# facebookresearch/multipathnet

Hardware: AMD Instinct MI355X
Metric: proposals/sec (1000 ROIs, 600x1000 img) VGG-16 Fast R-CNN (higher is better)
Workload: dtype f32; 1 GPU; VGG-16 Fast R-CNN, 1 image 600x1000 x 1000 ROIs per GPU per step, 21 classes, NMS 0.3, top-100 (BASELINE configs[1]); host image + boxes uploaded inside the step (pinned, copy stream, three staging sets)

## Files before the change

multipathnet_amd/csrc/dense.hip:

```cpp
#include <cstdlib>
#include <type_traits>
#include <vector>

#include "dense.h"

namespace mpn {

typedef float f32x16 __attribute__((ext_vector_type(16)));
typedef float f32x4 __attribute__((ext_vector_type(4)));

#define MPN_GPTR(p) ((const __attribute__((address_space(1))) void *)(p))
#define MPN_LPTR(p) ((__attribute__((address_space(3))) void *)(p))

__device__ __forceinline__ void glds16(const float *gsrc, float *lds_wave_base) {
  __builtin_amdgcn_global_load_lds(MPN_GPTR(gsrc), MPN_LPTR(lds_wave_base), 16, 0, 0);
}

__device__ __forceinline__ void glds16_saddr(const float *base_uniform, unsigned lane_byte_off, unsigned lds_byte_addr_uniform) {
  asm volatile("s_mov_b32 m0, %0\n\ts_nop 0\n\tglobal_load_lds_dwordx4 %1, %2"
               :
               : "s"(lds_byte_addr_uniform), "v"(lane_byte_off), "s"(base_uniform)
               : "memory");
}
__device__ __forceinline__ void dma_wait_all() { asm volatile("s_waitcnt vmcnt(0)" ::: "memory"); }
// ... 101 lines not shown
    if (MPN_ABLATE(a.ablate & 4)) {
#pragma unroll
      for (int mi = 0; mi < MI; ++mi) af[1][mi] = af[0][mi];
#pragma unroll
      for (int ni = 0; ni < NI; ++ni) bf[1][ni] = bf[0][ni];
    }
#pragma unroll
    for (int t = 0; t < TPS; ++t) {
      const int cur = t & 1;
      if (t + 1 < TPS && !MPN_ABLATE(a.ablate & 4)) {
        const int nt = t + 1, dy = (TPS == 9) ? nt / 3 : 0, dx = nt % 3;
#pragma unroll
        for (int mi = 0; mi < MI; ++mi) af[cur ^ 1][mi] = *reinterpret_cast<const f32x4 *>(Wl + (nt * BM + mbase + mi * 32) * 8);
#pragma unroll
        for (int ni = 0; ni < NI; ++ni) bf[cur ^ 1][ni] = *reinterpret_cast<const f32x4 *>(Il + ((rbase + ni + dy) * 34 + dx) * 8);
      }
      if (more) {
#pragma unroll
        for (int k = 0; k < PER_TAP; ++k) issue_item(q + 1, t * PER_TAP + k);
      }
      __builtin_amdgcn_sched_barrier(0);
#pragma unroll
      for (int j = 0; j < 4; ++j)
#pragma unroll
        for (int mi = 0; mi < MI; ++mi)
#pragma unroll
          for (int ni = 0; ni < NI; ++ni)
            acc[mi][ni] = __builtin_amdgcn_mfma_f32_32x32x2f32(af[cur][mi][j], bf[cur][ni][j], acc[mi][ni], 0, 0, 0);
      __builtin_amdgcn_sched_barrier(0);
    }
    if (!MPN_ABLATE(a.ablate & 2)) __syncthreads();
  }

  const int x = x0 + l31;
  const bool xok = x < a.W;
  if (a.splits > 1) {
    float *pb = a.part + (size_t)blockIdx.y * a.part_slab;
#pragma unroll
    for (int mi = 0; mi < MI; ++mi)
#pragma unroll
      for (int g = 0; g < 4; ++g) {
        const int cb = (cout0 + mbase + mi * 32) / 8 + g;
        if (cb >= a.out_cb) continue;
#pragma unroll
        for (int ni = 0; ni < NI; ++ni) {
          const int y = y0 + rbase + ni;
          if (xok && y < a.H) {
            f32x4 v;
#pragma unroll
            for (int e = 0; e < 4; ++e) v[e] = acc[mi][ni][g * 4 + e];
            *reinterpret_cast<f32x4 *>(pb + (size_t)cb * a.out_plane + ((size_t)(y + 1) * a.out_Wp + x + 1) * 8 + half * 4) = v;
          }
        }
      }
    return;
  }
  if (MPN_ABLATE(a.ablate & 8)) {
    if (a.H < 0) {
#pragma unroll
      for (int mi = 0; mi < MI; ++mi)
#pragma unroll
        for (int ni = 0; ni < NI; ++ni) *reinterpret_cast<f32x16 *>(a.part + (size_t)(mi * NI + ni) * 16 + lane * 64) = acc[mi][ni];
    }
    return;
  }
#pragma unroll
  for (int mi = 0; mi < MI; ++mi) {
#pragma unroll
    for (int g = 0; g < 4; ++g) {
      const int cb = (cout0 + mbase + mi * 32) / 8 + g;
      if (cb >= a.out_cb) continue;
      const f32x4 b4 = *reinterpret_cast<const f32x4 *>(a.bpk + cb * 8 + half * 4);
      f32x4 v[NI];
#pragma unroll
      for (int ni = 0; ni < NI; ++ni) {
        const int y = y0 + rbase + ni;
        const bool ok = xok && (y < a.H);
#pragma unroll
        for (int e = 0; e < 4; ++e) {
          float t = acc[mi][ni][g * 4 + e] + b4[e];
          if (a.relu) t = t < 0.0f ? 0.0f : t;
          v[ni][e] = t;
        }
        if (ok && a.out)
          *reinterpret_cast<f32x4 *>(a.out + (size_t)cb * a.out_plane + ((size_t)(y + 1) * a.out_Wp + x + 1) * 8 + half * 4) = v[ni];
        if (!ok) v[ni] = f32x4{-INFINITY, -INFINITY, -INFINITY, -INFINITY};
      }
      if constexpr (NI % 2 == 0) {
        if (a.pool) {
#pragma unroll
          for (int q = 0; q < NI / 2; ++q) {
            f32x4 m;
#pragma unroll
            for (int e = 0; e < 4; ++e) {
              float t = fmaxf(v[2 * q][e], v[2 * q + 1][e]);
              t = fmaxf(t, __shfl_xor(t, 1));
              m[e] = t > -INFINITY ? t : -INFINITY;
            }
            const int py = ((y0 + rbase) >> 1) + q, px = x >> 1;
            if (!(l31 & 1) && py < a.pool_H && px < a.pool_W)
              *reinterpret_cast<f32x4 *>(a.pool + (size_t)cb * a.pool_plane + ((size_t)(py + 1) * a.pool_Wp + px + 1) * 8 + half * 4) = m;
          }
        }
      }
    }
  }
}

MPN_KNOB(int, g_gemm_ablate, 0);

constexpr int kF_TH = 8;
constexpr int kF_PL = (kF_TH + 2) * 34 + 12;
template <int ABL>
__global__ __launch_bounds__(256, 5) void conv3x3_first_kernel(const float *__restrict__ in, int in_Wp, const float *__restrict__ w36,
                                                               int CoutP, const float *__restrict__ bpk, float *__restrict__ out,
                                                               size_t out_plane, int out_Wp, int H, int W, int out_cb, int relu,
                                                               int tiles_x, int n_tiles) {
  __shared__ float tile[2][4 * kF_PL];
  __shared__ float wl[36 * 64];
  __shared__ float bl[64];
  const int tid = threadIdx.x, lane = tid & 63;
  const int wave = __builtin_amdgcn_readfirstlane(tid >> 6);
  const int half = lane >> 5, l31 = lane & 31;
  const int cout0 = blockIdx.y * 64;
  for (int i = tid; i < 36 * 64; i += 256) wl[i] = w36[(size_t)(i >> 6) * CoutP + cout0 + (i & 63)];
  if (tid < 64) bl[tid] = bpk[cout0 + tid];
  constexpr int NPX = (kF_TH + 2) * 34;
  const int p0 = tid, p1 = tid + 256;
  const int r0 = p0 / 34, c0 = p0 - r0 * 34, r1 = p1 / 34, c1 = p1 - r1 * 34;
  const int off0 = (r0 * in_Wp + c0) * 8, off1 = p1 < NPX ? (r1 * in_Wp + c1) * 8 : off0;
  auto fetch = [&](int t, f32x4 &v0, f32x4 &v1) {
    const int ty = t / tiles_x, tx = t - ty * tiles_x;
    const float *base = in + ((size_t)(ty * kF_TH) * in_Wp + tx * 32) * 8;
    v0 = *reinterpret_cast<const f32x4 *>(base + off0);
    v1 = *reinterpret_cast<const f32x4 *>(base + off1);
  };
  auto park = [&](int buf, const f32x4 &v0, const f32x4 &v1) {
#pragma unroll
    for (int e = 0; e < 4; ++e) tile[buf][e * kF_PL + p0] = v0[e];
    if (p1 < NPX) {
#pragma unroll
      for (int e = 0; e < 4; ++e) tile[buf][e * kF_PL + p1] = v1[e];
    }
  };
  int t = blockIdx.x;
  if (t >= n_tiles) return;
  const int step = gridDim.x;
  f32x4 n0, n1;
  fetch(t, n0, n1);
  park(0, n0, n1);
  if (t + step < n_tiles) fetch(t + step, n0, n1);
  __syncthreads();
  const float *wa = wl + half * 64 + l31;
  int buf = 0;
  for (; t < n_tiles; t += step, buf ^= 1) {
    const int ty = t / tiles_x, tx = t - ty * tiles_x;
    const int y0 = ty * kF_TH, x0 = tx * 32;
    const float *tb = tile[buf] + half * kF_PL + (wave * 2) * 34 + l31;
    const int x = x0 + l31;
    bool xok = x < W;
    if constexpr ((ABL & 1) != 0) xok = xok && in_Wp == 7;
    const int yw = y0 + wave * 2;
    const unsigned voff = (unsigned)(((yw + 1) * out_Wp + x + 1) * 8 + half * 4) * 4u;
    const unsigned vrow = (unsigned)out_Wp * 32u;
    const bool ok0 = xok && yw < H, ok1 = xok && yw + 1 < H;
#pragma unroll
    for (int mi = 0; mi < 2; ++mi) {
      f32x16 acc[2];
#pragma unroll
      for (int ni = 0; ni < 2; ++ni)
#pragma unroll
        for (int r = 0; r < 16; ++r) acc[ni][r] = 0.0f;
#pragma unroll
      for (int tp = 0; tp < 9; ++tp) {
        const int dy = tp / 3, dx = tp - dy * 3;
#pragma unroll
        for (int p = 0; p < 2; ++p) {
          const float afr = wa[(tp * 2 + p) * 128 + mi * 32];
          float bfr[2];
#pragma unroll
          for (int ni = 0; ni < 2; ++ni) bfr[ni] = tb[2 * p * kF_PL + (ni + dy) * 34 + dx];
#pragma unroll
          for (int ni = 0; ni < 2; ++ni) {
            if constexpr ((ABL & 2) == 0) acc[ni] = __builtin_amdgcn_mfma_f32_32x32x2f32(afr, bfr[ni], acc[ni], 0, 0, 0);
            else acc[ni][(tp + p) & 15] += afr * bfr[ni];
          }
        }
        if ((tp % 3) == 2) __builtin_amdgcn_sched_barrier(0);
      }
      if (mi == 1) {
        const int tn = t + step;
        if (tn < n_tiles) {
          park(buf ^ 1, n0, n1);
          if (tn + step < n_tiles) fetch(tn + step, n0, n1);
        }
        __builtin_amdgcn_sched_barrier(0);
      }
#pragma unroll
      for (int g = 0; g < 4; ++g) {
        const int cb = __builtin_amdgcn_readfirstlane((cout0 + mi * 32) / 8 + g);
        if (cb >= out_cb) continue;
        const f32x4 b4 = *reinterpret_cast<const f32x4 *>(bl + (mi * 4 + g) * 8 + half * 4);
        char *pb = reinterpret_cast<char *>(out + (size_t)cb * out_plane);
#pragma unroll
        for (int ni = 0; ni < 2; ++ni) {
          f32x4 v;
#pragma unroll
          for (int e = 0; e < 4; ++e) {
            float tv = acc[ni][g * 4 + e] + b4[e];
            if (relu) tv = tv < 0.0f ? 0.0f : tv;
            v[e] = tv;
          }
          if (ni ? ok1 : ok0) *reinterpret_cast<f32x4 *>(pb + (voff + (ni ? vrow : 0u))) = v;
        }
      }
      __builtin_amdgcn_sched_barrier(0);
    }
    __syncthreads();
  }
}

__global__ void pack_conv_w_first_kernel(const float *__restrict__ w, int Cin, int Cout, int CoutP, float *__restrict__ w36) {
  const int t = blockIdx.x * blockDim.x + threadIdx.x;
  if (t >= 36 * CoutP) return;
  const int row = t / CoutP, co = t - row * CoutP;
  const int hf = row & 1, ks = row >> 1, p = ks & 1, tap = ks >> 1;
  const int cin = 2 * p + hf;
  w36[t] = (co < Cout && cin < Cin) ? w[((size_t)co * Cin + cin) * 9 + tap] : 0.0f;
}

size_t conv_first_elems(int Cout) { return (size_t)36 * conv_coutp(Cout); }

int pack_conv_weights_first(const float *d_w, int Cin, int Cout, float *d_w36, hipStream_t s) {
  MPN_CHECK_ARG(d_w && d_w36 && Cin > 0 && Cin <= 4 && Cout > 0);
  const int CoutP = conv_coutp(Cout);
  hipLaunchKernelGGL(pack_conv_w_first_kernel, dim3(cdiv(36 * CoutP, 256)), dim3(256), 0, s, d_w, Cin, Cout, CoutP, d_w36);
  MPN_CHECK_LAUNCH();
  return MPN_OK;
}

int conv3x3_first_c8p(Act in, const float *d_w36, const float *d_bpk, int Cout, int relu, Act out, hipStream_t s) {
  MPN_CHECK_ARG(in.p && d_w36 && d_bpk && out.p && in.C <= 4 && out.H == in.H && out.W == in.W && out.C == Cout);
  const int tiles_x = cdiv(in.W, 32), tiles_y = cdiv(in.H, kF_TH), n_ct = cdiv(Cout, 64);
  const int n_tiles = tiles_x * tiles_y;
  const char *e_cap = MPN_ABLATE(1) ? getenv("MPN_FIRST_BLOCKS") : nullptr;
  const int cap = e_cap ? atoi(e_cap) : 1280;
  const int blocks = cdiv(n_tiles, cdiv(n_tiles, cap));
  auto kern = conv3x3_first_kernel<0>;
#ifdef MPN_DEBUG_HOOKS
  if ((g_gemm_ablate & 3) == 1) kern = conv3x3_first_kernel<1>;
  if ((g_gemm_ablate & 3) == 2) kern = conv3x3_first_kernel<2>;
  if ((g_gemm_ablate & 3) == 3) kern = conv3x3_first_kernel<3>;
#endif
  hipLaunchKernelGGL(kern, dim3((unsigned)blocks, (unsigned)n_ct), dim3(256), 0, s, in.p, in.Wp, d_w36, conv_coutp(Cout), d_bpk, out.p,
                     out.plane(), out.Wp, in.H, in.W, (Cout + 7) / 8, relu, tiles_x, n_tiles);
  MPN_CHECK_LAUNCH();
  return MPN_OK;
}

template <int BM, int TH, int WM, int WN, int TPS>
static int launch_conv(const ConvArgs &a0, int tiles_y, hipStream_t s) {
  ConvArgs a = a0;
  constexpr int IN_LOADS = ((TH + 2) * 68 + 63) / 64;
  constexpr size_t LDS = (size_t)2 * (IN_LOADS * 256 + TPS * BM * 8) * sizeof(float);
  auto kern = conv3x3_c8p_kernel<BM, TH, WM, WN, TPS>;
  { int rc_attr = set_max_dyn_lds(reinterpret_cast<const void *>(kern), (int)LDS); if (rc_attr) return rc_attr; }
  dim3 grid((unsigned)(a.n_ct * tiles_y * a.tiles_x), (unsigned)a.splits);
  hipLaunchKernelGGL(kern, grid, dim3(256), LDS, s, a);
  MPN_CHECK_LAUNCH();
  return MPN_OK;
}


typedef float f32x2 __attribute__((ext_vector_type(2)));
__device__ __forceinline__ f32x2 pk_sub(f32x2 a, f32x2 b) {
  f32x2 r;
  asm("v_pk_add_f32 %0, %1, %2 neg_lo:[0,1] neg_hi:[0,1]" : "=v"(r) : "v"(a), "v"(b));
  return r;
}
__device__ __forceinline__ f32x2 vmax_2(f32x2 a, f32x2 b) {
  f32x2 r;
  asm("v_max_f32 %0, %1, %2" : "=v"(r[0]) : "v"(a[0]), "v"(b[0]));
  asm("v_max_f32 %0, %1, %2" : "=v"(r[1]) : "v"(a[1]), "v"(b[1]));
  return r;
}
__device__ __forceinline__ f32x2 vrelu_2(f32x2 a) {
  f32x2 r;
  asm("v_max_f32 %0, 0, %1" : "=v"(r[0]) : "v"(a[0]));
  asm("v_max_f32 %0, 0, %1" : "=v"(r[1]) : "v"(a[1]));
  return r;
}
__device__ __forceinline__ f32x2 vmax3_2(f32x2 a, f32x2 b, f32x2 c) {
  f32x2 r;
  asm("v_max3_f32 %0, %1, %2, %3" : "=v"(r[0]) : "v"(a[0]), "v"(b[0]), "v"(c[0]));
  asm("v_max3_f32 %0, %1, %2, %3" : "=v"(r[1]) : "v"(a[1]), "v"(b[1]), "v"(c[1]));
  return r;
}
__device__ __forceinline__ f32x2 vmax3_2s(f32x2 a, f32x2 b, float c_uniform) {
  f32x2 r;
  asm("v_max3_f32 %0, %1, %2, %3" : "=v"(r[0]) : "v"(a[0]), "v"(b[0]), "s"(c_uniform));
  asm("v_max3_f32 %0, %1, %2, %3" : "=v"(r[1]) : "v"(a[1]), "v"(b[1]), "s"(c_uniform));
  return r;
}
constexpr int WG_RAW_LOADS = 12;
constexpr int WG_RAW_FLOATS = WG_RAW_LOADS * 256;
constexpr int WG_V_FLOATS = 16 * 64 * 8;
constexpr int WG_U_FLOATS = 16 * 64 * 8;
constexpr size_t WG_LDS_BYTES = (size_t)2 * (WG_RAW_FLOATS + WG_V_FLOATS + WG_U_FLOATS) * sizeof(float);

template <int ABL, int TC>
__global__ __launch_bounds__(256) void conv3x3_wino_kernel(ConvArgs a) {
  constexpr int TR = 64 / TC;
  constexpr int RC = 2 * TC + 2, RR = 2 * TR + 2;
  constexpr int WG_RAW_PIECES = RR * RC * 2;
  static_assert((WG_RAW_PIECES + 63) / 64 <= WG_RAW_LOADS, "raw tile DMA slots");
  extern __shared__ __attribute__((aligned(16))) float lds[];
  float *const raw_lds = lds;
  float *const v_lds = lds + 2 * WG_RAW_FLOATS;
  float *const u_lds = v_lds + 2 * WG_V_FLOATS;
  const int tid = threadIdx.x, lane = tid & 63;
  unsigned long long tk0 = 0, tk1 = 0, tk2 = 0;
  if constexpr ((ABL & 64) != 0) tk0 = __builtin_amdgcn_s_memtime();
  const int wave = __builtin_amdgcn_readfirstlane(tid >> 6);
  const int half = lane >> 5, l31 = lane & 31;
  int bid = blockIdx.x, split = blockIdx.y, cps = a.chunks_per_split;
  bool partial = a.splits > 1;
  if (a.tail_splits > 1 && bid >= a.tail_first) {
    const int t = bid - a.tail_first;
    split = t % a.tail_splits; bid = a.tail_first + t / a.tail_splits; cps = a.tail_cps; partial = true;
  }
  const int ct = bid % a.n_ct, sp = bid / a.n_ct;
  const int tyb = sp / a.tiles_x, txb = sp - tyb * a.tiles_x;
  const int y0 = tyb * (2 * TR), x0 = txb * (2 * TC), cout0 = ct * 64;
  const int mbase = (wave >> 1) * 32, nbase = (wave & 1) * 32;

  constexpr int RAW_IT = (WG_RAW_LOADS + 3) / 4;
  unsigned raw_rel[RAW_IT];
#pragma unroll
  for (int i = 0; i < RAW_IT; ++i) {
    int p = min((i * 4 + wave) * 64 + lane, WG_RAW_PIECES - 1);
    int r = p / (RC * 2), o = p - r * (RC * 2);
    raw_rel[i] = (unsigned)(((r * a.in_Wp) * 8 + o * 4) * 4);
  }
  const unsigned u_lane = (unsigned)((((wave & 1) * 64 + lane) * 4) * 4);
  const size_t u_chunk = (size_t)16 * a.CoutP * 8;
  const float *const in_tile = a.in + (size_t)(y0 * a.in_Wp + x0) * 8;
  const float *const w_tile = a.wpk + (size_t)cout0 * 8;
  const unsigned lds0 = lds_byte_addr(lds);
  const unsigned raw_slot = lds0 + (unsigned)(wave * 256) * 4, u_slot = lds0 + (unsigned)(2 * WG_RAW_FLOATS + 2 * WG_V_FLOATS + wave * 256) * 4;
  auto issue_raw_item = [&](int c, int buf, int i) {
    glds16_saddr(in_tile + (size_t)c * a.in_plane, raw_rel[i], raw_slot + (unsigned)(buf * WG_RAW_FLOATS + i * 1024) * 4);
  };
  auto issue_raw = [&](int c, int buf) {
#pragma unroll
    for (int i = 0; i < RAW_IT; ++i) issue_raw_item(c, buf, i);
  };
  auto issue_u = [&](int c, int buf, int i) {
    const float *slice = w_tile + (size_t)c * u_chunk + (size_t)(((i * 4 + wave) >> 1) * a.CoutP) * 8;
    glds16_saddr(slice, u_lane, u_slot + (unsigned)(buf * WG_U_FLOATS + i * 1024) * 4);
  };

  const int tf_tile = wave * 16 + (lane >> 2), tf_cp = lane & 3;
  const int tf_rd = ((2 * (tf_tile / TC)) * RC + 2 * (tf_tile % TC)) * 8 + 2 * tf_cp;
  const int tf_wr = tf_tile * 8 + ((2 * tf_cp) ^ (((tf_tile >> 3) & 1) << 2));
  f32x2 d[16], t[16];
  auto tf_load = [&](int buf) {
    const float *R = raw_lds + buf * WG_RAW_FLOATS + tf_rd;
#pragma unroll
    for (int r = 0; r < 4; ++r)
#pragma unroll
      for (int q = 0; q < 4; ++q) d[r * 4 + q] = *reinterpret_cast<const f32x2 *>(R + (r * RC + q) * 8);
  };
  auto tf_rows = [&]() {
#pragma unroll
    for (int q = 0; q < 4; ++q) {
      t[0 + q] = d[0 + q] - d[8 + q];
      t[4 + q] = d[4 + q] + d[8 + q];
      t[8 + q] = d[8 + q] - d[4 + q];
      t[12 + q] = d[4 + q] - d[12 + q];
    }
  };
  auto tf_cols_store = [&](int xi, int buf) {
    float *Vw = v_lds + buf * WG_V_FLOATS + tf_wr + xi * 4 * 512;
    *reinterpret_cast<f32x2 *>(Vw + 0 * 512) = t[xi * 4 + 0] - t[xi * 4 + 2];
    *reinterpret_cast<f32x2 *>(Vw + 1 * 512) = t[xi * 4 + 1] + t[xi * 4 + 2];
    *reinterpret_cast<f32x2 *>(Vw + 2 * 512) = t[xi * 4 + 2] - t[xi * 4 + 1];
    *reinterpret_cast<f32x2 *>(Vw + 3 * 512) = t[xi * 4 + 1] - t[xi * 4 + 3];
  };

  auto tf_load_item = [&](int buf, int i) {
    const float *R = raw_lds + buf * WG_RAW_FLOATS + tf_rd + ((i >> 1) * RC + (i & 1) * 2) * 8;
    d[2 * i] = *reinterpret_cast<const f32x2 *>(R);
    d[2 * i + 1] = *reinterpret_cast<const f32x2 *>(R + 8);
  };
  auto tf_rows_item = [&](int q) {
    t[0 + q] = d[0 + q] - d[8 + q];
    t[4 + q] = d[4 + q] + d[8 + q];
    t[8 + q] = d[8 + q] - d[4 + q];
    t[12 + q] = d[4 + q] - d[12 + q];
  };
  auto tf_cols_compute = [&](int xi) {
    const f32x2 v0 = t[xi * 4 + 0] - t[xi * 4 + 2], v1 = t[xi * 4 + 1] + t[xi * 4 + 2];
    const f32x2 v2 = t[xi * 4 + 2] - t[xi * 4 + 1], v3 = t[xi * 4 + 1] - t[xi * 4 + 3];
    t[xi * 4 + 0] = v0; t[xi * 4 + 1] = v1; t[xi * 4 + 2] = v2; t[xi * 4 + 3] = v3;
  };
  auto tf_store_item = [&](int i, int buf) {
    float *Vw = v_lds + buf * WG_V_FLOATS + tf_wr + (2 * i) * 512;
    *reinterpret_cast<f32x2 *>(Vw) = t[2 * i];
    *reinterpret_cast<f32x2 *>(Vw + 512) = t[2 * i + 1];
  };

  const int c0 = split * cps;
  const int c1 = min(a.nchunks, c0 + cps);
  const int n_more = c1 - 1 - c0;
  const int b0 = n_more & 1;
  issue_raw(c0, b0);
#pragma unroll
  for (int i = 0; i < 8; ++i) issue_u(c0, b0, i);
  issue_raw(min(c0 + 1, c1 - 1), b0 ^ 1);
  f32x16 acc[16];
  if constexpr ((ABL & 128) == 0) dma_wait_all();
  __syncthreads();
  tf_load(b0);
  tf_rows();
#pragma unroll
  for (int xi = 0; xi < 4; ++xi) tf_cols_store(xi, b0);
  __syncthreads();

  const int frag_sw = (half ^ ((l31 >> 3) & 1)) * 4;
  const int frag_u = (mbase + l31) * 8 + frag_sw, frag_v = (nbase + l31) * 8 + frag_sw;
  f32x4 af[2][2], bf[2][2];
  auto load_frags = [&](int buf, int pr, int slot) {
    const float *Ul = u_lds + buf * WG_U_FLOATS + frag_u, *Vl = v_lds + buf * WG_V_FLOATS + frag_v;
#pragma unroll
    for (int k = 0; k < 2; ++k) {
      af[slot][k] = *reinterpret_cast<const f32x4 *>(Ul + (2 * pr + k) * 512);
      bf[slot][k] = *reinterpret_cast<const f32x4 *>(Vl + (2 * pr + k) * 512);
    }
  };
  load_frags(b0, 0, 0);
  unsigned long long tr0 = 0, tr1 = 0, tr2 = 0;
  auto body = [&](int c, auto more_tag, auto parity_tag, auto first_tag) {
    constexpr bool MORE = decltype(more_tag)::value;
    constexpr int s = decltype(parity_tag)::value;
    constexpr bool FIRST = decltype(first_tag)::value;
#pragma unroll
    for (int p = 0; p < 8; ++p) {
      const int cur = p & 1;
      if constexpr ((ABL & 64) != 0) {
        if (p == 0) tr0 = __builtin_amdgcn_s_memtime();
        if (a.trace && blockIdx.x < 4 && blockIdx.y == 0 && tid == 0 && (c - c0) == 5) a.trace[4 * 64 * 4 + blockIdx.x * 8 + p] = __builtin_amdgcn_s_memtime();
      }
      if (p == 7 && MORE) {
        if constexpr ((ABL & 64) != 0) tr1 = __builtin_amdgcn_s_memtime();
        __builtin_amdgcn_s_waitcnt(0xc07f);
        if constexpr ((ABL & 64) != 0) tr2 = __builtin_amdgcn_s_memtime();
        dma_wait_all();
        if constexpr (!(ABL & 2)) __syncthreads();
        if constexpr ((ABL & 64) != 0) {
          const unsigned long long tr3 = __builtin_amdgcn_s_memtime();
          if (a.trace && blockIdx.x < 4 && blockIdx.y == 0 && tid == 0) {
            unsigned long long *o = a.trace + ((size_t)blockIdx.x * 64 + (c - c0)) * 4;
            o[0] = tr0; o[1] = tr1 - tr0; o[2] = tr2 - tr1; o[3] = tr3 - tr2;
          }
        }
        if constexpr (!(ABL & 16)) load_frags(s ^ 1, 0, 0);
      }
#pragma unroll
      for (int i = 0; i < 8; ++i) {
        __builtin_amdgcn_sched_barrier(0);
        if constexpr (FIRST) {
          if (i < 2) acc[2 * p + (i & 1)] = __builtin_amdgcn_mfma_f32_32x32x2f32(af[cur][i & 1][0], bf[cur][i & 1][0], f32x16{}, 0, 0, 0);
        }
        if (!FIRST || i >= 2)
          acc[2 * p + (i & 1)] = __builtin_amdgcn_mfma_f32_32x32x2f32(af[cur][i & 1][i >> 1], bf[cur][i & 1][i >> 1], acc[2 * p + (i & 1)], 0, 0, 0);
        __builtin_amdgcn_sched_barrier(0);
        if (i == 0 && p + 1 < 8 && !(ABL & 16)) load_frags(s, p + 1, cur ^ 1);
        if constexpr (MORE) {
          const int m = p * 8 + i;
          if constexpr (!(ABL & 1)) {
            if (m >= 1 && m <= 8) issue_u(c + 1, s ^ 1, m - 1);
            else if (m >= 9 && m <= 11) issue_raw_item(min(c + 2, c1 - 1), s, m - 9);
          }
          if constexpr (!(ABL & 4)) {
            if (m >= 12 && m <= 19) tf_load_item(s ^ 1, m - 12);
            else if (m == 27) {
#pragma unroll
              for (int q = 0; q < 4; ++q) tf_rows_item(q);
#pragma unroll
              for (int xi = 0; xi < 4; ++xi) tf_cols_compute(xi);
            } else if (m >= 28 && m <= 35) tf_store_item(m - 28, s ^ 1);
          }
        }
      }
    }
  };
  if constexpr ((ABL & 64) != 0) tk1 = __builtin_amdgcn_s_memtime();
  using P0 = std::integral_constant<int, 0>;
  using P1 = std::integral_constant<int, 1>;
  using T = std::true_type;
  using F = std::false_type;
  f32x4 bias4[4];
  auto load_bias = [&]() {
#pragma unroll
    for (int g = 0; g < 4; ++g) {
      const int cb = min((cout0 + mbase) / 8 + g, a.out_cb - 1);
      bias4[g] = *reinterpret_cast<const f32x4 *>(a.bpk + cb * 8 + half * 4);
    }
  };
  if (n_more == 0) {
#pragma unroll
    for (int k = 0; k < 16; ++k)
#pragma unroll
      for (int r = 0; r < 16; ++r) acc[k][r] = 0.0f;
  } else {
    int cc = c0;
    if (n_more & 1) { body(cc, T{}, P1{}, T{}); ++cc; }
    else { body(cc, T{}, P0{}, T{}); body(cc + 1, T{}, P1{}, F{}); cc += 2; }
    for (; cc < c1 - 1; cc += 2) { body(cc, T{}, P0{}, F{}); body(cc + 1, T{}, P1{}, F{}); }
  }
  load_bias();
  body(c1 - 1, F{}, P0{}, F{});
#pragma unroll
  for (int g = 0; g < 4; ++g) asm volatile("" : "+v"(bias4[g]));
  if constexpr ((ABL & 64) != 0) tk2 = __builtin_amdgcn_s_memtime();

  if constexpr ((ABL & 8) != 0) {
    if (a.H < 0) {
#pragma unroll
      for (int k = 0; k < 16; ++k) *reinterpret_cast<f32x16 *>(a.part + (size_t)k * 16 + lane * 256) = acc[k];
    }
    return;
  }
  const int tau = nbase + l31;
  const int y = y0 + 2 * (tau / TC), x = x0 + 2 * (tau % TC);
  float *const obase = partial ? a.part + (size_t)split * a.part_slab : a.out;
  const unsigned off00 = (unsigned)((((y + 1) * a.out_Wp + x + 1) * 8 + half * 4) * 4);
  const unsigned row_b = (unsigned)(a.out_Wp * 32);
  const unsigned offk[4] = {off00, off00 + 32u, off00 + row_b, off00 + row_b + 32u};
  const int py = y >> 1, px = x >> 1;
  const unsigned offp = (unsigned)((((py + 1) * a.pool_Wp + px + 1) * 8 + half * 4) * 4);
  auto out_transform = [&](int g, f32x2 (&Y)[4][2]) {
#pragma unroll
    for (int ep = 0; ep < 2; ++ep) {
      const int r = g * 4 + ep * 2;
      f32x2 m[16];
#pragma unroll
      for (int k = 0; k < 16; ++k) {
        asm("v_accvgpr_read_b32 %0, %1" : "=v"(m[k][0]) : "a"(acc[k][r]));
        asm("v_accvgpr_read_b32 %0, %1" : "=v"(m[k][1]) : "a"(acc[k][r + 1]));
      }
      const f32x2 s0 = m[0] + m[4] + m[8], s1 = m[1] + m[5] + m[9], s2 = m[2] + m[6] + m[10], s3 = m[3] + m[7] + m[11];
      const f32x2 u0 = pk_sub(pk_sub(m[4], m[8]), m[12]), u1 = pk_sub(pk_sub(m[5], m[9]), m[13]);
      const f32x2 u2 = pk_sub(pk_sub(m[6], m[10]), m[14]), u3 = pk_sub(pk_sub(m[7], m[11]), m[15]);
      Y[0][ep] = s0 + s1 + s2; Y[1][ep] = pk_sub(pk_sub(s1, s2), s3);
      Y[2][ep] = u0 + u1 + u2; Y[3][ep] = pk_sub(pk_sub(u1, u2), u3);
    }
  };
  const int cb0 = (cout0 + mbase) / 8;
  const bool interior = y0 + 2 * TR <= a.H && x0 + 2 * TC <= a.W &&
                        (partial || !a.pool || ((y0 >> 1) + TR <= a.pool_H && (x0 >> 1) + TC <= a.pool_W));
  enum { FIN_EDGE, FIN_PARTIAL, FIN_POOLED, FIN_FULL };
  const int fin = !interior ? FIN_EDGE : partial ? FIN_PARTIAL : a.out == nullptr ? FIN_POOLED : FIN_FULL;
  const float ninf = -INFINITY;
  const bool okx1 = x + 1 < a.W, oky1 = y + 1 < a.H, ok00 = y < a.H && x < a.W;
  const bool okk[4] = {ok00, ok00 && okx1, ok00 && oky1, ok00 && okx1 && oky1};
  const bool okp = a.pool && py < a.pool_H && px < a.pool_W;
#pragma unroll
  for (int g = 0; g < 4; ++g) {
    const int cb = cb0 + g;
    if (cb >= a.out_cb) continue;
    f32x2 Y[4][2];
    out_transform(g, Y);
    const f32x2 b01 = f32x2{bias4[g][0], bias4[g][1]}, b23 = f32x2{bias4[g][2], bias4[g][3]};
    char *const ob = reinterpret_cast<char *>(obase + (size_t)cb * a.out_plane);
    char *const pb = reinterpret_cast<char *>(a.pool + (size_t)cb * a.pool_plane);
    if (fin == FIN_POOLED) {
      f32x2 v0 = vmax3_2s(vmax3_2(Y[0][0], Y[1][0], Y[2][0]), Y[3][0], ninf) + b01;
      f32x2 v1 = vmax3_2s(vmax3_2(Y[0][1], Y[1][1], Y[2][1]), Y[3][1], ninf) + b23;
      if (a.relu) { v0 = vrelu_2(v0); v1 = vrelu_2(v1); }
      if (a.pool) *reinterpret_cast<f32x4 *>(pb + offp) = f32x4{v0[0], v0[1], v1[0], v1[1]};
    } else if (fin == FIN_FULL) {
      f32x2 V[4][2];
#pragma unroll
      for (int k = 0; k < 4; ++k) { V[k][0] = Y[k][0] + b01; V[k][1] = Y[k][1] + b23; }
      if (a.relu) {
#pragma unroll
        for (int k = 0; k < 4; ++k) { V[k][0] = vrelu_2(V[k][0]); V[k][1] = vrelu_2(V[k][1]); }
      }
#pragma unroll
      for (int k = 0; k < 4; ++k) *reinterpret_cast<f32x4 *>(ob + offk[k]) = f32x4{V[k][0][0], V[k][0][1], V[k][1][0], V[k][1][1]};
      if (a.pool) {
        const f32x2 mx0 = vmax3_2s(vmax3_2(V[0][0], V[1][0], V[2][0]), V[3][0], ninf), mx1 = vmax3_2s(vmax3_2(V[0][1], V[1][1], V[2][1]), V[3][1], ninf);
        *reinterpret_cast<f32x4 *>(pb + offp) = f32x4{mx0[0], mx0[1], mx1[0], mx1[1]};
      }
    } else if (fin == FIN_PARTIAL) {
#pragma unroll
      for (int k = 0; k < 4; ++k) *reinterpret_cast<f32x4 *>(ob + offk[k]) = f32x4{Y[k][0][0], Y[k][0][1], Y[k][1][0], Y[k][1][1]};
    } else if (partial) {
#pragma unroll
      for (int k = 0; k < 4; ++k)
        if (okk[k]) *reinterpret_cast<f32x4 *>(ob + offk[k]) = f32x4{Y[k][0][0], Y[k][0][1], Y[k][1][0], Y[k][1][1]};
    } else {
      f32x2 mx0 = f32x2{-INFINITY, -INFINITY}, mx1 = mx0;
#pragma unroll
      for (int k = 0; k < 4; ++k) {
        f32x2 v0 = Y[k][0] + b01, v1 = Y[k][1] + b23;
        if (a.relu) { v0 = vrelu_2(v0); v1 = vrelu_2(v1); }
        if (okk[k] && a.out) *reinterpret_cast<f32x4 *>(ob + offk[k]) = f32x4{v0[0], v0[1], v1[0], v1[1]};
        if (okk[k]) { mx0 = vmax_2(mx0, v0); mx1 = vmax_2(mx1, v1); }
      }
      if (okp) *reinterpret_cast<f32x4 *>(pb + offp) = f32x4{mx0[0], mx0[1], mx1[0], mx1[1]};
    }
    __builtin_amdgcn_sched_barrier(0);
  }
  if constexpr ((ABL & 64) != 0) {
    const unsigned long long tk3 = __builtin_amdgcn_s_memtime();
    if (a.trace && blockIdx.x < 4 && blockIdx.y == 0 && tid == 0) {
      unsigned long long *o = a.trace + 4 * 64 * 4 + 32 + blockIdx.x * 4;
      o[0] = tk1 - tk0; o[1] = tk2 - tk1; o[2] = tk3 - tk2; o[3] = tk0;
    }
    if (a.trace && blockIdx.y == 0 && tid == 0 && blockIdx.x < 4096) {
      unsigned long long *o = a.trace + 4 * 64 * 4 + 48 + (size_t)blockIdx.x * 3;
      const unsigned hw = __builtin_amdgcn_s_getreg((31 << 11) | 4), xcc = __builtin_amdgcn_s_getreg((31 << 11) | 20);
      o[0] = ((unsigned long long)xcc << 32) | hw; o[1] = tk0; o[2] = tk3;
    }
  }
}

template <int ABL>
static int launch_conv_wino_t(const ConvArgs &a, int tiles_y, hipStream_t s) {
  auto kern = a.wino_tc == 16 ? conv3x3_wino_kernel<ABL, 16> : conv3x3_wino_kernel<ABL, 8>;
  { int rc_attr = set_max_dyn_lds(reinterpret_cast<const void *>(kern), (int)WG_LDS_BYTES); if (rc_attr) return rc_attr; }
  const int blocks = a.n_ct * tiles_y * a.tiles_x;
  dim3 grid((unsigned)(a.tail_splits > 1 ? a.tail_first + (blocks - a.tail_first) * a.tail_splits : blocks), (unsigned)a.splits);
  hipLaunchKernelGGL(kern, grid, dim3(256), WG_LDS_BYTES, s, a);
  MPN_CHECK_LAUNCH();
  return MPN_OK;
}

static int launch_conv_wino(const ConvArgs &a, int tiles_y, hipStream_t s) {
#ifdef MPN_DEBUG_HOOKS
  switch (a.ablate) {
    case 1: return launch_conv_wino_t<1>(a, tiles_y, s);
    case 2: return launch_conv_wino_t<2>(a, tiles_y, s);
    case 4: return launch_conv_wino_t<4>(a, tiles_y, s);
    case 8: return launch_conv_wino_t<8>(a, tiles_y, s);
    case 5: return launch_conv_wino_t<5>(a, tiles_y, s);
    case 23: return launch_conv_wino_t<23>(a, tiles_y, s);
    case 31: return launch_conv_wino_t<31>(a, tiles_y, s);
    case 64: return launch_conv_wino_t<64>(a, tiles_y, s);
    case 128: return launch_conv_wino_t<128>(a, tiles_y, s);
    case 136: return launch_conv_wino_t<136>(a, tiles_y, s);
    default: break;
  }
#endif
  return launch_conv_wino_t<0>(a, tiles_y, s);
}

__global__ void conv_splitk_reduce_kernel(const float *__restrict__ part, size_t slab, int S, size_t plane, int Wp, int H, int W,
                                          int out_cb, const float *__restrict__ bpk, int relu, float *__restrict__ out,
                                          float *__restrict__ pool, size_t pool_plane, int pool_Wp, int pool_H, int pool_W,
                                          int tile_first, int tiles_x, int g_start, int th_log, int tw_log) {
  const bool pooling = pool != nullptr;
  const int GHf = pooling ? pool_H : H, GW = pooling ? pool_W : W;
  const int GH = GHf - g_start;
  size_t t = (size_t)blockIdx.x * blockDim.x + threadIdx.x;
  size_t total = (size_t)out_cb * GH * GW * 2;
  if (t >= total) return;
  const int h = (int)(t & 1); size_t r = t >> 1;
  const int gx = (int)(r % GW); r /= GW;
  const int gy = g_start + (int)(r % GH); const int cb = (int)(r / GH);
  if (tile_first > 0) {
    const int ty = (pooling ? 2 * gy : gy) >> th_log, tx = (pooling ? 2 * gx : gx) >> tw_log;
    if (ty * tiles_x + tx < tile_first) return;
  }
  const f32x4 b4 = *reinterpret_cast<const f32x4 *>(bpk + cb * 8 + h * 4);
  f32x4 m = f32x4{-INFINITY, -INFINITY, -INFINITY, -INFINITY};
  const int ny = pooling ? 2 : 1, nx = pooling ? 2 : 1;
  for (int dy = 0; dy < ny; ++dy)
    for (int dx = 0; dx < nx; ++dx) {
      const int y = pooling ? 2 * gy + dy : gy, x = pooling ? 2 * gx + dx : gx;
      if (y >= H || x >= W) continue;
      const size_t off = (size_t)cb * plane + ((size_t)(y + 1) * Wp + x + 1) * 8 + h * 4;
      f32x4 v = *reinterpret_cast<const f32x4 *>(part + off);
      for (int s = 1; s < S; ++s) v += *reinterpret_cast<const f32x4 *>(part + s * slab + off);
      v += b4;
      if (relu) {
#pragma unroll
        for (int e = 0; e < 4; ++e) v[e] = relu == 2 ? fmaxf(v[e], 0.0f) : (v[e] < 0.0f ? 0.0f : v[e]);
      }
      if (out) *reinterpret_cast<f32x4 *>(out + off) = v;
#pragma unroll
      for (int e = 0; e < 4; ++e) m[e] = v[e] > m[e] ? v[e] : m[e];
    }
  if (pooling) *reinterpret_cast<f32x4 *>(pool + (size_t)cb * pool_plane + ((size_t)(gy + 1) * pool_Wp + gx + 1) * 8 + h * 4) = m;
}

MPN_KNOB(unsigned long long *, g_wino_trace, nullptr);
MPN_KNOB(int, g_conv_split, 0);

static int conv_pick_splits(int blocks, int nchunks, int slots) {
  if (g_conv_split > 0) return g_conv_split < nchunks ? g_conv_split : nchunks;
  if (g_conv_split < 0) return 1;
  auto fill = [&](int b) { return (double)b / ((double)slots * ((b + slots - 1) / slots)); };
  int best = 1;
  double best_score = fill(blocks);
  for (int S = 2; S <= 8; ++S) {
    if (nchunks / S < 6) break;
    double score = fill(blocks * S) * (1.0 - 0.04 - 0.01 * S);
    if (score > best_score * 1.08) { best_score = score; best = S; }
  }
  return best;
}

static int wino_pick_splits(int blocks, int nchunks, size_t out_bytes) {
  if (g_conv_split > 0) return g_conv_split < nchunks ? g_conv_split : nchunks;
  if (g_conv_split < 0) return 1;
  const double t_chunk = 4740.0, t_ovh = 14000.0, hz = 2.35e9;
  int best = 1;
  double best_t = 1e30;
  for (int S = 1; S <= 8 && S <= nchunks; ++S) {
    const int cps = (nchunks + S - 1) / S;
    const int Se = (nchunks + cps - 1) / cps;
    if (Se != S) continue;
    const long long rounds = ((long long)blocks * S + 255) / 256;
    double t = rounds * (cps * t_chunk + t_ovh);
    if (S > 1) t += ((S + 1) * (double)out_bytes / 8.0e12 + 3e-6) * hz;
    if (t < best_t * 0.995) { best_t = t; best = S; }
  }
  return best;
}

struct WinoPlan { int splits, tail_first, tail_splits, tail_cps; };
static WinoPlan wino_pick_plan(int blocks, int n_ct, int nchunks, size_t out_bytes) {
  WinoPlan p{1, 0, 0, 0};
  if (g_conv_split < 0) {
    const int S = -g_conv_split < nchunks ? -g_conv_split : nchunks;
    const int first = (blocks / 2 / n_ct) * n_ct;
    if (S > 1 && first > 0 && first < blocks) {
      p.tail_cps = cdiv(nchunks, S); p.tail_splits = cdiv(nchunks, p.tail_cps); p.tail_first = first;
      if (p.tail_splits < 2) p = WinoPlan{1, 0, 0, 0};
    }
    return p;
  }
  p.splits = wino_pick_splits(blocks, nchunks, out_bytes);
  if (g_conv_split > 0) return p;
  const double t_chunk = 4740.0, t_ovh = 14000.0, hz = 2.35e9;
  auto t_uniform = [&](int S) {
    const int cps = cdiv(nchunks, S);
    const long long rounds = ((long long)blocks * cdiv(nchunks, cps) + 255) / 256;
    double t = rounds * (cps * t_chunk + t_ovh);
    if (S > 1) t += ((S + 1) * (double)out_bytes / 8.0e12 + 3e-6) * hz;
    return t;
  };
  double best_t = t_uniform(p.splits);
  const int full = (blocks / 256) * 256 / n_ct * n_ct, rem = blocks - full;
  if (full > 0 && rem > 0) {
    const double tile_bytes = 64.0 * 256.0 * 4.0;
    for (int S = 2; S <= 8 && S <= nchunks / 2; ++S) {
      const int cps = cdiv(nchunks, S), Se = cdiv(nchunks, cps);
      if (Se != S) continue;
      const long long rounds = ((long long)rem * S + 255) / 256;
      const double t = (double)(full / 256) * (nchunks * t_chunk + t_ovh) + rounds * (cps * t_chunk + t_ovh) +
                       ((S + 1) * rem * tile_bytes / 8.0e12 + 3e-6) * hz;
      if (t < best_t * 0.98) { best_t = t; p = WinoPlan{1, full, S, cps}; }
    }
  }
  return p;
}

MPN_KNOB(int, g_wino_tc, 0);
MPN_KNOB(int, g_conv_variant, 0);

#ifdef MPN_DEBUG_HOOKS
static int g_conv_last_plan[8];
static void record_conv_plan(int variant, const ConvArgs &a, bool reduce) {
  const int v[8] = {variant, a.wino_tc, a.splits, a.chunks_per_split, a.tail_first, a.tail_splits, a.tail_cps, reduce ? 1 : 0};
  for (int i = 0; i < 8; ++i) g_conv_last_plan[i] = v[i];
}
#define MPN_RECORD_CONV_PLAN(variant, a, reduce) record_conv_plan(variant, a, reduce)
#else
#define MPN_RECORD_CONV_PLAN(variant, a, reduce) ((void)0)
#endif

int conv3x3_variant_for(int Cout, bool has_wino) {
  int variant = g_conv_variant & 15;
  if (variant == 7 && !has_wino) variant = 0;
  if (variant == 0) variant = has_wino ? 7 : ((Cout <= 64) ? 2 : 1);
  return variant;
}

int conv3x3_c8p(Act in, const float *d_wpk, const float *d_bpk, int Cout, int relu, Act out, Act pooled, hipStream_t s, const float *d_wino,
                bool batch_invariant) {
  MPN_CHECK_ARG(in.p && (d_wpk || d_wino) && d_bpk && (out.p || pooled.p));
  ConvArgs a{};
  a.in = in.p; a.in_plane = in.plane(); a.in_Wp = in.Wp;
  a.wpk = d_wpk; a.CoutP = conv_coutp(Cout); a.bpk = d_bpk;
  a.out = out.p; a.out_plane = out.p ? out.plane() : 0; a.out_Wp = out.p ? out.Wp : 0;
  a.pool = pooled.p; a.pool_plane = pooled.p ? pooled.plane() : 0; a.pool_Wp = pooled.p ? pooled.Wp : 0;
  a.pool_H = pooled.p ? pooled.H : 0; a.pool_W = pooled.p ? pooled.W : 0;
  a.H = in.H; a.W = in.W; a.nchunks = in.Cb(); a.out_cb = (Cout + 7) / 8; a.relu = relu;
  a.tiles_x = cdiv(in.W, 32);
  a.ablate = g_gemm_ablate;
  a.trace = g_wino_trace;
  if (out.p) MPN_CHECK_ARG(out.H == in.H && out.W == in.W && out.C == Cout);
  if (pooled.p) MPN_CHECK_ARG(pooled.H == (in.H + 1) / 2 && pooled.W == (in.W + 1) / 2 && pooled.C == Cout);
  int variant = conv3x3_variant_for(Cout, d_wino != nullptr);
  if (!d_wpk) variant = 7;
  if (variant == 7) {
    a.wpk = d_wino;
    const long px_sq = (long)cdiv(in.H, 16) * 16 * cdiv(in.W, 16) * 16, px_wide = (long)cdiv(in.H, 8) * 8 * cdiv(in.W, 32) * 32;
    a.wino_tc = batch_invariant ? 16 : (g_wino_tc == 8 || g_wino_tc == 16) ? g_wino_tc : (px_wide < px_sq ? 16 : 8);
    const int tpx_h = a.wino_tc == 16 ? 8 : 16, tpx_w = a.wino_tc == 16 ? 32 : 16;
    a.tiles_x = cdiv(in.W, tpx_w);
    const int tiles_y = cdiv(in.H, tpx_h);
    a.n_ct = cdiv(Cout, 64);
    const int blocks = a.n_ct * tiles_y * a.tiles_x;
    Act geo = out.p ? out : make_act(nullptr, Cout, in.H, in.W);
    const WinoPlan plan = batch_invariant ? WinoPlan{1, 0, 0, 0} : wino_pick_plan(blocks, a.n_ct, a.nchunks, geo.elems() * sizeof(float));
    a.splits = plan.splits;
    a.chunks_per_split = cdiv(a.nchunks, a.splits);
    a.splits = cdiv(a.nchunks, a.chunks_per_split);
    a.tail_first = plan.tail_first; a.tail_splits = plan.tail_splits; a.tail_cps = plan.tail_cps;
    const int n_slabs = a.tail_splits > 1 ? a.tail_splits : a.splits;
    if (n_slabs > 1) {
      a.part_slab = geo.elems();
      a.out_plane = geo.plane(); a.out_Wp = geo.Wp;
      size_t need = a.part_slab * n_slabs * sizeof(float);
      void *ws = nullptr;
      { int rc_ws = scratch_get(SCR_CONV_SPLITK, need, s, &ws); if (rc_ws) return rc_ws; }
      a.part = static_cast<float *>(ws);
    }
    MPN_RECORD_CONV_PLAN(7, a, n_slabs > 1);
    int rc = launch_conv_wino(a, tiles_y, s);
    if (rc != MPN_OK || n_slabs == 1) return rc;
    const int GH = pooled.p ? pooled.H : in.H, GW = pooled.p ? pooled.W : in.W;
    int tile_first = 0, g_start = 0;
    if (a.tail_splits > 1) {
      tile_first = a.tail_first / a.n_ct;
      const int y_start = (tile_first / a.tiles_x) * tpx_h;
      g_start = pooled.p ? y_start / 2 : y_start;
    }
    const size_t total = (size_t)a.out_cb * (GH - g_start) * GW * 2;
    hipLaunchKernelGGL(conv_splitk_reduce_kernel, dim3((unsigned)cdiv_sz(total, 256)), dim3(256), 0, s, a.part, a.part_slab, n_slabs, geo.plane(),
                       geo.Wp, in.H, in.W, a.out_cb, d_bpk, relu ? 2 : 0, out.p, pooled.p, a.pool_plane, a.pool_Wp, a.pool_H, a.pool_W, tile_first,
                       a.tiles_x, g_start, a.wino_tc == 16 ? 3 : 4, a.wino_tc == 16 ? 5 : 4);
    MPN_CHECK_LAUNCH();
    return MPN_OK;
  }
  const bool wide = (variant == 1 || variant == 3 || variant == 5);
  const int th = variant == 5 ? 8 : (variant == 6 ? 16 : (wide ? 4 : 8));
  const int tiles_y = cdiv(in.H, th);
  a.n_ct = cdiv(Cout, wide ? 128 : 64);
  const int blocks = a.n_ct * tiles_y * a.tiles_x;
  const int slots = (variant == 1 || variant >= 5) ? 256 : (variant == 2 ? 512 : 768);
  a.splits = conv_pick_splits(blocks, a.nchunks, slots);
  a.chunks_per_split = cdiv(a.nchunks, a.splits);
  a.splits = cdiv(a.nchunks, a.chunks_per_split);
  Act geo = out.p ? out : make_act(nullptr, Cout, in.H, in.W);
  if (a.splits > 1) {
    a.part_slab = geo.elems();
    a.out_plane = geo.plane(); a.out_Wp = geo.Wp;
    size_t need = a.part_slab * a.splits * sizeof(float);
    void *ws = nullptr;
    { int rc_ws = scratch_get(SCR_CONV_SPLITK, need, s, &ws); if (rc_ws) return rc_ws; }
    a.part = static_cast<float *>(ws);
  }
  MPN_RECORD_CONV_PLAN(variant, a, a.splits > 1);
  int rc;
  switch (variant) {
    case 1: rc = launch_conv<128, 4, 2, 2, 9>(a, tiles_y, s); break;
    case 2: rc = launch_conv<64, 8, 1, 4, 9>(a, tiles_y, s); break;
    case 3: rc = launch_conv<128, 4, 2, 2, 3>(a, tiles_y, s); break;
    case 5: rc = launch_conv<128, 8, 2, 2, 9>(a, tiles_y, s); break;
    case 6: rc = launch_conv<64, 16, 1, 4, 9>(a, tiles_y, s); break;
    default: rc = launch_conv<64, 8, 1, 4, 3>(a, tiles_y, s); break;
  }
  if (rc != MPN_OK || a.splits == 1) return rc;
  const int GH = pooled.p ? pooled.H : in.H, GW = pooled.p ? pooled.W : in.W;
  const size_t total = (size_t)a.out_cb * GH * GW * 2;
  hipLaunchKernelGGL(conv_splitk_reduce_kernel, dim3((unsigned)cdiv_sz(total, 256)), dim3(256), 0, s, a.part, a.part_slab, a.splits, geo.plane(),
                     geo.Wp, in.H, in.W, a.out_cb, d_bpk, relu ? 1 : 0, out.p, pooled.p, a.pool_plane, a.pool_Wp, a.pool_H, a.pool_W, 0, 0, 0, 4, 4);
  MPN_CHECK_LAUNCH();
  return MPN_OK;
}

struct GemmArgs {
  const float *x; int Mp;
  const float *wpk; int NP;
  const float *bpk;
  float *y;
  int M, nstages, stages_per_split, relu, n_mt, n_nt, direct;
  int seg_stages;
  int n_fast;
  const float *res;
  int nsb, sb0, sb1;
  const float *rs0, *rs1, *rs2;
  int rs_mod;
  int xp;
  int bin_rows, out_Mp;
  unsigned long long *trace;
};

template <int KCH, bool FOLD, bool RSI = false, bool TRACE = false>
__global__ __launch_bounds__(256) void gemm_c8_pf_kernel(GemmArgs a) {
  static_assert(!(FOLD && RSI), "row scales are applied either through the running total or in place");
  static_assert(!TRACE || KCH == 4, "the trace record holds the chunk starts of a 4-chunk stage");
  unsigned long long tk0 = 0, tk1 = 0, tk2 = 0;
  if constexpr (TRACE) tk0 = __builtin_amdgcn_s_memtime();
  constexpr int OP_FLOATS = KCH * 128 * 8;
  constexpr int STAGE = 2 * OP_FLOATS;
  constexpr int IT = OP_FLOATS / 256 / 4;
  extern __shared__ __attribute__((aligned(16))) float lds[];
  const int tid = threadIdx.x, lane = tid & 63;
  const int wave = __builtin_amdgcn_readfirstlane(tid >> 6);
  const int half = lane >> 5, l31 = lane & 31;
  int b = blockIdx.x;
  const int nb = gridDim.x;
  {
    const int per = nb >> 3, rem = nb & 7, xcd = b & 7, idx = b >> 3;
    b = xcd < rem ? xcd * (per + 1) + idx : rem * (per + 1) + (xcd - rem) * per + idx;
  }
  const int nt = a.n_fast ? b % a.n_nt : b / a.n_mt, mt = a.n_fast ? b / a.n_nt : b - nt * a.n_mt;
  const int n0 = nt * 128, m0 = mt * 128;
  const int split = blockIdx.y;
  const int st0 = split * a.stages_per_split;
  const int st1 = min(a.nstages, st0 + a.stages_per_split);
  const int wm = wave >> 1, wn = wave & 1;

  static_assert(IT == KCH, "one 1-KiB wave-load per wave per K chunk per operand");
  const unsigned dma_piece = (unsigned)(wave * 64 + lane);
  const unsigned dma_lane = (dma_piece ^ ((dma_piece >> 4) & 1u)) * 16u;
  const size_t a_stage = (size_t)KCH * a.NP * 8, b_stage = (size_t)KCH * a.xp * 8;
  const float *const a_tile = a.wpk + (size_t)n0 * 8, *const b_tile = a.x + (size_t)m0 * 8;
  const unsigned lds0 = lds_byte_addr(lds) + (unsigned)(wave * 256) * 4;
  auto issue_a = [&](int st, int s, int i) {
    glds16_saddr(a_tile + (size_t)st * a_stage + (size_t)i * a.NP * 8, dma_lane, lds0 + (unsigned)(s * STAGE + i * 1024) * 4);
  };
  auto issue_b = [&](int st, int s, int i) {
    glds16_saddr(b_tile + (size_t)st * b_stage + (size_t)i * a.xp * 8, dma_lane, lds0 + (unsigned)(s * STAGE + OP_FLOATS + i * 1024) * 4);
  };

  f32x16 acc[2][2];
#pragma unroll
  for (int mi = 0; mi < 2; ++mi)
#pragma unroll
    for (int ni = 0; ni < 2; ++ni)
#pragma unroll
      for (int r = 0; r < 16; ++r) acc[mi][ni][r] = 0.0f;

// ... 1869 lines not shown
```

Baseline: 303,100 proposals/s.

## Re-spread Winograd conv DMA, transform and fragment loads across MFMA slots

Reschedules the software pipeline inside the Winograd conv main loop. The per-chunk DMA issues, transform loads, stores and transform arithmetic move to a new table of MFMA slot positions, spread more evenly through the 64 MFMAs. Fragment loads for the next pair are split into four single-register loads interleaved after MFMAs 4-7, and the next chunk's first fragments are prefetched during the last pair instead of after the barrier. Weight-slice DMA now uses precomputed scalar offsets. The aim is to hide LDS and global latency behind matrix math and shorten the stall at the chunk boundary, at the risk of more register pressure and LDS hazards.

```diff
diff --git a/multipathnet_amd/csrc/dense.hip b/multipathnet_amd/csrc/dense.hip
--- a/multipathnet_amd/csrc/dense.hip
+++ b/multipathnet_amd/csrc/dense.hip
@@ -427,6 +427,12 @@
   asm("v_max3_f32 %0, %1, %2, %3" : "=v"(r[1]) : "v"(a[1]), "v"(b[1]), "s"(c_uniform));
   return r;
 }
+enum { WS_DMA, WS_LOAD, WS_WRITE };
+constexpr int WS_ARITH = 36;
+constexpr int wino_slot(int kind, int j) {
+  const int dma[11] = {0, 1, 2, 3, 8, 9, 10, 11, 16, 17, 18}, load[8] = {19, 24, 25, 26, 27, 32, 33, 34}, store[8] = {40, 41, 42, 43, 48, 49, 50, 51};
+  return kind == WS_DMA ? dma[j] : kind == WS_LOAD ? load[j] : store[j];
+}
 constexpr int WG_RAW_LOADS = 12;
 constexpr int WG_RAW_FLOATS = WG_RAW_LOADS * 256;
 constexpr int WG_V_FLOATS = 16 * 64 * 8;
@@ -563,12 +569,19 @@
       bf[slot][k] = *reinterpret_cast<const f32x4 *>(Vl + (2 * pr + k) * 512);
     }
   };
+  auto load_frag = [&](int buf, int pr, int slot, int j) {
+    const int k = j >> 1;
+    if ((j & 1) == 0) af[slot][k] = *reinterpret_cast<const f32x4 *>(u_lds + buf * WG_U_FLOATS + frag_u + (2 * pr + k) * 512);
+    else bf[slot][k] = *reinterpret_cast<const f32x4 *>(v_lds + buf * WG_V_FLOATS + frag_v + (2 * pr + k) * 512);
+  };
   load_frags(b0, 0, 0);
   unsigned long long tr0 = 0, tr1 = 0, tr2 = 0;
   auto body = [&](int c, auto more_tag, auto parity_tag, auto first_tag) {
     constexpr bool MORE = decltype(more_tag)::value;
     constexpr int s = decltype(parity_tag)::value;
     constexpr bool FIRST = decltype(first_tag)::value;
+    size_t u_off = 0;
+    const float *raw_src = nullptr;
 #pragma unroll
     for (int p = 0; p < 8; ++p) {
       const int cur = p & 1;
@@ -589,7 +602,6 @@
             o[0] = tr0; o[1] = tr1 - tr0; o[2] = tr2 - tr1; o[3] = tr3 - tr2;
           }
         }
-        if constexpr (!(ABL & 16)) load_frags(s ^ 1, 0, 0);
       }
 #pragma unroll
       for (int i = 0; i < 8; ++i) {
@@ -600,21 +612,48 @@
         if (!FIRST || i >= 2)
           acc[2 * p + (i & 1)] = __builtin_amdgcn_mfma_f32_32x32x2f32(af[cur][i & 1][i >> 1], bf[cur][i & 1][i >> 1], acc[2 * p + (i & 1)], 0, 0, 0);
         __builtin_amdgcn_sched_barrier(0);
-        if (i == 0 && p + 1 < 8 && !(ABL & 16)) load_frags(s, p + 1, cur ^ 1);
+        if constexpr (!(ABL & 16)) {
+          if (i >= 4 && p + 1 < 8) load_frag(s, p + 1, cur ^ 1, i - 4);
+          else if (i < 4 && p == 7 && MORE) load_frag(s ^ 1, 0, 0, i);
+        }
         if constexpr (MORE) {
           const int m = p * 8 + i;
           if constexpr (!(ABL & 1)) {
-            if (m >= 1 && m <= 8) issue_u(c + 1, s ^ 1, m - 1);
-            else if (m >= 9 && m <= 11) issue_raw_item(min(c + 2, c1 - 1), s, m - 9);
+#pragma unroll
+            for (int j = 0; j < 11; ++j)
+              if (m == wino_slot(WS_DMA, j)) {
+                if (j == 0) {
+                  int cn = c + 1;
+                  asm volatile("" : "+s"(cn));
+                  u_off = (size_t)cn * u_chunk * sizeof(float);
+                }
+                if (j == 8) {
+                  int cr = min(c + 2, c1 - 1);
+                  asm volatile("" : "+s"(cr));
+                  raw_src = in_tile + (size_t)cr * a.in_plane;
+                }
+                if (j < 8) {
+                  asm volatile("" : "+s"(u_off));
+                  const float *slice0 = w_tile + (size_t)(((j * 4 + wave) >> 1) * a.CoutP) * 8;
+                  glds16_saddr(reinterpret_cast<const float *>(reinterpret_cast<const char *>(slice0) + u_off), u_lane,
+                               u_slot + (unsigned)((s ^ 1) * WG_U_FLOATS + j * 1024) * 4);
+                } else {
+                  glds16_saddr(raw_src, raw_rel[j - 8], raw_slot + (unsigned)(s * WG_RAW_FLOATS + (j - 8) * 1024) * 4);
+                }
+              }
           }
           if constexpr (!(ABL & 4)) {
-            if (m >= 12 && m <= 19) tf_load_item(s ^ 1, m - 12);
-            else if (m == 27) {
+#pragma unroll
+            for (int j = 0; j < 8; ++j) {
+              if (m == wino_slot(WS_LOAD, j)) tf_load_item(s ^ 1, j);
+              if (m == wino_slot(WS_WRITE, j)) tf_store_item(j, s ^ 1);
+            }
+            if (m == WS_ARITH) {
 #pragma unroll
               for (int q = 0; q < 4; ++q) tf_rows_item(q);
 #pragma unroll
               for (int xi = 0; xi < 4; ++xi) tf_cols_compute(xi);
-            } else if (m >= 28 && m <= 35) tf_store_item(m - 28, s ^ 1);
+            }
           }
         }
       }
@@ -771,7 +810,9 @@
     case 2: return launch_conv_wino_t<2>(a, tiles_y, s);
     case 4: return launch_conv_wino_t<4>(a, tiles_y, s);
     case 8: return launch_conv_wino_t<8>(a, tiles_y, s);
-    case 5: return launch_conv_wino_t<5>(a, tiles_y, s);
+    case 16: return launch_conv_wino_t<16>(a, tiles_y, s);
+    case 20: return launch_conv_wino_t<20>(a, tiles_y, s);
+    case 5:return launch_conv_wino_t<5>(a, tiles_y, s);
     case 23: return launch_conv_wino_t<23>(a, tiles_y, s);
     case 31: return launch_conv_wino_t<31>(a, tiles_y, s);
     case 64: return launch_conv_wino_t<64>(a, tiles_y, s);
```

After: 305,300 proposals/s (median of 6 runs). About the same (+0.8%).
